# zhenyuw16/Uni3DETR

Hardware: AMD Instinct MI355X
Metric: scenes/sec (fwd+bwd) SUN-RGB-D 20k pts, 300 queries (higher is better)
Workload: dtype bf16

## Files before the change

include/u3d_hip.h:

```cpp
#ifndef U3D_HIP_H_
#define U3D_HIP_H_

#include <stddef.h>
#include <stdint.h>

#ifdef __cplusplus
extern "C" {
#endif

typedef struct ihipStream_t* u3d_stream;

enum {
  U3D_OK = 0,
  U3D_ERR_ARG = -1,
  U3D_ERR_UNSUPPORTED = -2,
  U3D_ERR_LAUNCH = -3,
  U3D_ERR_WORKSPACE = -4
};

enum { U3D_F32 = 0, U3D_BF16 = 1 };

int32_t u3d_version(void);
const char* u3d_strerror(int32_t code);

// ... 54 lines not shown
                           const int32_t* n_out_dev, int32_t n_out_cap, int32_t cin, int32_t cout, int32_t kvol,
                           int32_t transpose_w, u3d_stream s);
int32_t u3d_igemm_fwd_add_bf16(const void* in, const void* w, const int32_t* nbr, int32_t ld, const void* addend, void* out,
                               const int32_t* n_out_dev, int32_t n_out_cap, int32_t cin, int32_t cout, int32_t kvol,
                               int32_t transpose_w, u3d_stream s);
int32_t u3d_linear_bf16(const void* x, const void* w, const float* bias, int32_t relu, void* out, const int32_t* m_dev,
                        int32_t m_cap, int32_t k, int32_t n, u3d_stream s);
int64_t u3d_bn_fold_job_bytes(void);
int32_t u3d_bn_fold_job_blocks(int32_t kvol, int32_t cout, int32_t cin);
int32_t u3d_bn_fold_batched(const void* jobs, int32_t njobs, int32_t total_blocks, u3d_stream s);
int32_t u3d_igemm_fwd_affine_bf16(const void* in, const void* w_folded, const int32_t* nbr, int32_t ld, const float* shift, int32_t relu,
                                  void* out, const int32_t* n_out_dev, int32_t n_out_cap, int32_t cin, int32_t cout, int32_t kvol,
                                  u3d_stream s);
int32_t u3d_igemm_fwd_affine_plan(int32_t n_out_cap, int32_t cin, int32_t cout, int32_t kvol, int32_t has_nbr, int32_t* kernel,
                                  int32_t* rows, int32_t* cols);
int32_t u3d_igemm_fwd_split_bf16(const void* in, const void* w, const int32_t* nbr, int32_t ld, float* out, const int32_t* n_out_dev,
                                 int32_t n_out_cap, int32_t cin, int32_t cout, int32_t kvol3, double* stats, const float* addend, u3d_stream s);
int32_t u3d_igemm_direct_split_bf16(const void* in, const void* w3, const int32_t* nbr, int32_t ld, float* out, const int32_t* n_out_dev,
                                    int32_t n_out_cap, int32_t n_in_cap, int32_t cin, int32_t cout, u3d_stream s);
int32_t u3d_split3_weights(const float* src, int64_t sk, int64_t sa, int64_t sb, int32_t k, int32_t a, int32_t b, void* dst, u3d_stream s);
typedef struct U3dSplitRowsJobs {
  const float* src[32];
  void* dst[32];
  int32_t ld[32], rows[32], cols[32];
  int32_t first_block[33];
  int32_t njobs;
} U3dSplitRowsJobs;
int32_t u3d_split_rows_batch(const U3dSplitRowsJobs* jobs, u3d_stream s);
int32_t u3d_sum3_f32(const float* a, const float* b, const float* c, float* out, int64_t n, u3d_stream s);
int64_t u3d_split3_job_bytes(void);
int32_t u3d_split3_job_blocks(int32_t k, int32_t a, int32_t b);
int32_t u3d_split3_weights_batch(const void* jobs, int32_t njobs, int32_t total_blocks, u3d_stream s);
int32_t u3d_split_rows_f32(const float* x, const int32_t* n_dev, int32_t n_cap, int32_t c, void* dst, u3d_stream s);
int32_t u3d_igemm_fwd_stats_bf16(const void* in, const void* w, const int32_t* nbr, int32_t ld, void* out,
                                 const int32_t* n_out_dev, int32_t n_out_cap, int32_t cin, int32_t cout, int32_t kvol,
                                 double* stats, u3d_stream s);
int32_t u3d_igemm_fwd_stats_layout(int32_t n_out_cap, int32_t cin, int32_t cout, int32_t kvol, int32_t has_nbr, int32_t* partials,
                                   int32_t* rows_per_partial);
typedef struct {
  const void* x;
  const void* y;
  const float* mean;
  const float* invstd;
  const float* gamma;
  const float* beta;
  int32_t relu;
  int32_t reserved;
} u3d_bn_epi;
int32_t u3d_igemm_dgrad_bnstats_bf16(const void* in, const void* w, const int32_t* nbr, int32_t ld, const void* addend, void* out,
                                     const int32_t* n_out_dev, int32_t n_out_cap, int32_t cin, int32_t cout, int32_t kvol,
                                     const u3d_bn_epi* bn, double* stats, u3d_stream s);
int32_t u3d_bn_bwd_finalize_partials(const double* partial, int32_t nblocks, int32_t rows_per_block, const int32_t* n_dev,
                                     int32_t n_cap, int32_t c, double* sums, float* sums_f32, u3d_stream s);
int32_t u3d_subm_halo_sizes(int32_t n_cap, int64_t* tile_rows_elems, int64_t* loc_elems, int32_t* tiles);
int32_t u3d_subm_halo_build(const int32_t* nbr, int32_t ld, const int32_t* n_dev, int32_t n_cap, int32_t* tile_rows,
                            uint16_t* loc, int32_t* tile_cnt, int32_t kvol, u3d_stream s);
int32_t u3d_subm_halo_wpack(const void* w_nmajor, void* w_packed, u3d_stream s);
int32_t u3d_subm_halo_wpack_batched(const void* const* srcs_dev, void* const* dsts_dev, int32_t n, u3d_stream s);
int32_t u3d_subm_halo_conv64_bf16(const void* in, const void* w_packed, const int32_t* tile_rows, const uint16_t* loc,
                                  const int32_t* tile_cnt, const int32_t* n_dev, int32_t n_cap, int32_t krev,
                                  const void* addend, void* out, double* stats, const u3d_bn_epi* bn, int32_t max_slots,
                                  u3d_stream s);
int32_t u3d_subm_halo_wpack128(const void* w_nmajor, void* w_packed, int32_t kvol, u3d_stream s);
int32_t u3d_subm_halo_wpack128_batched(const void* const* srcs_dev, void* const* dsts_dev, int32_t n, int32_t kvol, u3d_stream s);
int32_t u3d_subm_halo_conv128_bf16(const void* in, const void* w_packed, const int32_t* tile_rows, const uint16_t* loc,
                                   const int32_t* tile_cnt, const int32_t* n_dev, int32_t n_cap, int32_t krev,
                                   const void* addend, void* out, double* stats, int32_t max_slots, int32_t kvol, u3d_stream s);
int64_t u3d_subm_halo_wgrad64_workspace(void);
int32_t u3d_subm_halo_wgrad64_bf16(const void* x, const void* dy, const int32_t* tile_rows, const uint16_t* loc,
                                   const int32_t* tile_cnt, const int32_t* n_dev, int32_t n_cap, float* dw, void* workspace,
                                   int64_t workspace_bytes, int32_t max_slots, u3d_stream s);
int64_t u3d_igemm_wgrad_bf16_workspace(int32_t n_out_cap, int32_t cin, int32_t cout, int32_t kvol);
int32_t u3d_igemm_wgrad_bf16(const void* in, const void* dout, const int32_t* nbr, int32_t ld, float* dw,
                             const int32_t* n_out_dev, int32_t n_out_cap, int32_t cin, int32_t cout, int32_t kvol,
                             int32_t out_layout, void* workspace, int64_t workspace_bytes, u3d_stream s);
int32_t u3d_igemm_wgrad_plan(int32_t n_out_cap, int32_t cin, int32_t cout, int32_t kvol, int32_t has_nbr, int32_t out_layout,
                             int32_t* kernel, int32_t* tile, int32_t* nsplit, int64_t* workspace);

int64_t u3d_spconv_wgrad_workspace(int32_t n_out_cap, int32_t cin, int32_t cout, int32_t kvol);
int32_t u3d_spconv_wgrad(const void* in, const void* dout, const int32_t* nbr, int32_t ld, float* dw,
                         const int32_t* n_out_dev, int32_t n_out_cap, int32_t cin, int32_t cout, int32_t kvol,
                         int32_t dtype, void* workspace, int64_t workspace_bytes, u3d_stream s);

int64_t u3d_colsum_workspace(int32_t n, int32_t c);
int32_t u3d_colsum(const void* x, int32_t n, int32_t c, int32_t dtype, float* out, void* workspace,
                   int64_t workspace_bytes, u3d_stream s);

int64_t u3d_wgrad_batched_workspace(int32_t count, int32_t n_rows, int32_t cin, int32_t cout);
int32_t u3d_wgrad_batched_bf16(const void* const* in, const void* const* dout, float* const* dw, int32_t count,
                               const int32_t* n_dev, int32_t n_rows, int32_t cin, int32_t cout, void* workspace,
                               int64_t workspace_bytes, u3d_stream s);
int64_t u3d_colsum_batched_workspace(int32_t count, int32_t n, int32_t c);
int32_t u3d_colsum_batched(const void* const* x, float* const* out, int32_t count, int32_t n, int32_t c, int32_t dtype,
                           void* workspace, int64_t workspace_bytes, u3d_stream s);

int32_t u3d_skinny_wgrad_chunks(int32_t m);
int32_t u3d_skinny_wgrad_bf16(const void* dy, const void* x, int32_t m, int32_t n, int32_t k, float* partial, u3d_stream s);
int32_t u3d_skinny_wgrad_batched(const void* const* dy, const void* const* x, float* const* partial, const int32_t* n, const int32_t* k,
                                 int32_t count, int32_t m, int32_t dy_skinny, u3d_stream s);

int64_t u3d_bn_stats_workspace(int32_t n_cap, int32_t c);
int32_t u3d_bn_stats(const void* x, const int32_t* n_dev, int32_t n_cap, int32_t c, int32_t dtype,
                     double* sums, void* workspace, int64_t workspace_bytes, u3d_stream s);
int32_t u3d_bn_finalize(const double* sums, const int32_t* n_dev, int32_t n_cap, int32_t c, float eps, float momentum,
                        float* running_mean, float* running_var, int64_t* num_batches, float* mean, float* invstd,
                        u3d_stream s);
// ... 367 lines not shown
```

uni3detr_amd/native.py:

```python
import ctypes as C
import os

import numpy as np
import torch

_HERE = os.path.dirname(os.path.abspath(__file__))
LIB_PATH = os.environ.get("U3D_LIB_PATH") or os.path.join(_HERE, "libu3d_hip.so")

F32, BF16 = 0, 1


class U3DError(RuntimeError):
    pass


class BitGridStruct(C.Structure):
    _fields_ = [("words", C.c_void_p), ("prefix", C.c_void_p), ("batch", C.c_int32), ("dz", C.c_int32),
                ("dy", C.c_int32), ("dx", C.c_int32), ("layout", C.c_int32), ("row_capacity", C.c_int32)]


DL_NLIN, DL_NLN = 22, 7
(DL_RPH0, DL_RPH1, DL_RPH2, DL_QS0, DL_QS1, DL_QS2, DL_INQK, DL_INV, DL_OUTP, DL_OPROJ, DL_PE1, DL_FFN0, DL_FFN1, DL_REG0, DL_REG1,
 DL_REG2, DL_CLS0, DL_CLS1, DL_CLS2, DL_IOU0, DL_IOU1, DL_IOU2) = range(DL_NLIN)
(DLN_1, DLN_2, DLN_3, DLN_PE0, DLN_PE1, DLN_C1, DLN_C2) = range(DL_NLN)
# ... 18 lines not shown
    _fields_ = [("src", C.c_void_p), ("dst", C.c_void_p), ("dst_t", C.c_void_p), ("n", C.c_int32), ("k", C.c_int32),
                ("n_pad", C.c_int32), ("n_pad_t", C.c_int32), ("t_plain", C.c_int32), ("reserved", C.c_int32)]


_lib = None
_P = C.c_void_p
_I = C.c_int32
_L = C.c_int64
_I3 = C.c_int32 * 3
_F3 = C.c_float * 3
_F6 = C.c_float * 6

_SIGS = {
    "u3d_version": (_I, []),
    "u3d_strerror": (C.c_char_p, [_I]),
    "u3d_points_augment": (_I, [_P, _P, _I, _I, _I, _P, _I, _I, _P]),
    "u3d_boxes_augment": (_I, [_P, _P, _I, _I, _I, _P, _I, _P]),
    "u3d_points_range_filter": (_I, [_P, _P, _I, _I, C.POINTER(C.c_float), _P, _P, _P]),
    "u3d_point_sample": (_I, [_P, _P, _P, _I, _I, _I, _P, _P, _P, _P]),
    "u3d_boxes_range_filter": (_I, [_P, _P, _P, _I, _I, C.POINTER(C.c_float), _P, _P]),
    "u3d_point_shuffle": (_I, [_P, _P, _P, _I, _I, _I, _P, _P, _P]),
    "u3d_boxes_label_filter": (_I, [_P, _P, _P, _P, _I, _I, _I, _P, _P]),
    "u3d_batch_ingest": (_I, [_P, _I, _I, _P, _P, _I, _I, _P, _I, _I, _P, _P, _P, _I, _I, _P, _P, _P, _P, _P, _P, _P, _P]),
    "u3d_sweeps_merge_workspace": (_L, [_I]),
    "u3d_sweeps_merge": (_I, [_P, _L, _P, _L, _I, _P, _P, _I, _P, _P, _I, _I, C.POINTER(C.c_int32), _I, _I, _P, _L, _P, _L, _P, _P]),
    "u3d_event_create": (_I, [C.POINTER(C.c_void_p)]),
    "u3d_event_record": (_I, [C.c_void_p, _I, _P]),
    "u3d_event_elapsed_ms": (_I, [C.c_void_p, C.c_void_p, C.POINTER(C.c_float)]),
    "u3d_event_destroy": (_I, [C.c_void_p]),
    "u3d_bitgrid_nwords": (_L, [_I, _I, _I, _I]),
    "u3d_bitgrid_nwords_layout": (_L, [_I, _I, _I, _I, _I]),
    "u3d_voxelize_dynamic": (_I, [_P, _P, _I, _I, _I, _F3, _F6, _P, _P]),
    "u3d_scatter_mean": (_I, [_P, _P, _I, _I, _P, _P, _I, _P]),
    "u3d_bitgrid_mark": (_I, [C.POINTER(BitGridStruct), _P, _I, _P]),
    "u3d_bitgrid_mark_strided": (_I, [C.POINTER(BitGridStruct), _P, _P, _I, _I3, _I3, _I3, _P]),
    "u3d_bitgrid_scan_scratch": (_L, [_L]),
    "u3d_bitgrid_scan": (_I, [C.POINTER(BitGridStruct), _P, _P]),
    "u3d_bitgrid_rank": (_I, [C.POINTER(BitGridStruct), _P, _I, _P, _P]),
    "u3d_bitgrid_coords": (_I, [C.POINTER(BitGridStruct), _P, _I, _P]),
    "u3d_nbr_table": (_I, [C.POINTER(BitGridStruct), _P, _P, _I, _I3, _I3, _I3, _I, _P, _I, _P]),
    "u3d_dense_nbr_table": (_I, [_I, _I3, _I3, _I3, _I3, _I3, _I, _P, _I, _P]),
    "u3d_voxelize_hard_workspace": (_L, [_I, _I, _I]),
    "u3d_voxelize_hard": (_I, [_P, _P, _I, _I, _I, _I, _F3, _F6, _I, _I, _P, _P, _P, _P, _P, _P, _L, _P]),
    "u3d_spconv_fwd": (_I, [_P, _P, _P, _I, _P, _P, _I, _I, _I, _I, _I, _I, _P]),
    "u3d_spconv_wgrad_workspace": (_L, [_I, _I, _I, _I]),
    "u3d_spconv_wgrad": (_I, [_P, _P, _P, _I, _P, _P, _I, _I, _I, _I, _I, _P, _L, _P]),
    "u3d_igemm_fwd_bf16": (_I, [_P, _P, _P, _I, _P, _P, _I, _I, _I, _I, _I, _P]),
    "u3d_igemm_fwd_stats_layout": (_I, [_I, _I, _I, _I, _I, _P, _P]),
    "u3d_igemm_fwd_add_bf16": (_I, [_P, _P, _P, _I, _P, _P, _P, _I, _I, _I, _I, _I, _P]),
    "u3d_linear_bf16": (_I, [_P, _P, _P, _I, _P, _P, _I, _I, _I, _P]),
    "u3d_igemm_wgrad_bf16_workspace": (_L, [_I, _I, _I, _I]),
    "u3d_igemm_wgrad_bf16": (_I, [_P, _P, _P, _I, _P, _P, _I, _I, _I, _I, _I, _P, _L, _P]),
    "u3d_igemm_wgrad_plan": (_I, [_I, _I, _I, _I, _I, _I, _P, _P, _P, _P]),
    "u3d_colsum_workspace": (_L, [_I, _I]),
    "u3d_colsum": (_I, [_P, _I, _I, _I, _P, _P, _L, _P]),
    "u3d_bn_stats_workspace": (_L, [_I, _I]),
    "u3d_bn_stats": (_I, [_P, _P, _I, _I, _I, _P, _P, _L, _P]),
    "u3d_bn_finalize": (_I, [_P, _P, _I, _I, C.c_float, C.c_float, _P, _P, _P, _P, _P, _P]),
    "u3d_bn_forward_stats": (_I, [_P, _P, _I, _I, _I, C.c_float, C.c_float, _P, _P, _P, _P, _P, _P, _L, _P]),
    "u3d_bn_finalize_partials": (_I, [_P, _I, _I, _P, _I, _I, C.c_float, C.c_float, _P, _P, _P, _P, _P, _P]),
    "u3d_igemm_fwd_stats_bf16": (_I, [_P, _P, _P, _I, _P, _P, _I, _I, _I, _I, _P, _P]),
    "u3d_igemm_fwd_split_bf16": (_I, [_P, _P, _P, _I, _P, _P, _I, _I, _I, _I, _P, _P, _P]),
    "u3d_split_rows_f32": (_I, [_P, _P, _I, _I, _P, _P]),
    "u3d_split3_weights": (_I, [_P, C.c_int64, C.c_int64, C.c_int64, _I, _I, _I, _P, _P]),
    "u3d_sum3_f32": (_I, [_P, _P, _P, _P, C.c_int64, _P]),
    "u3d_split_rows_batch": (_I, [_P, _P]),
    "u3d_split3_job_bytes": (C.c_int64, []),
    "u3d_split3_job_blocks": (_I, [_I, _I, _I]),
    "u3d_split3_weights_batch": (_I, [_P, _I, _I, _P]),
    "u3d_bn_fold_job_bytes": (C.c_int64, []),
    "u3d_bn_fold_job_blocks": (_I, [_I, _I, _I]),
    "u3d_bn_fold_batched": (_I, [_P, _I, _I, _P]),
    "u3d_igemm_fwd_affine_bf16": (_I, [_P, _P, _P, _I, _P, _I, _P, _P, _I, _I, _I, _I, _P]),
    "u3d_igemm_fwd_affine_plan": (_I, [_I, _I, _I, _I, _I, _P, _P, _P]),
    "u3d_igemm_direct_split_bf16": (_I, [_P, _P, _P, _I, _P, _P, _I, _I, _I, _I, _P]),
    "u3d_igemm_dgrad_bnstats_bf16": (_I, [_P, _P, _P, _I, _P, _P, _P, _I, _I, _I, _I, _P, _P, _P]),
    "u3d_bn_bwd_finalize_partials": (_I, [_P, _I, _I, _P, _I, _I, _P, _P, _P]),
    "u3d_subm_halo_sizes": (_I, [_I, _P, _P, _P]),
    "u3d_subm_halo_build": (_I, [_P, _I, _P, _I, _P, _P, _P, _I, _P]),
    "u3d_subm_halo_wpack128": (_I, [_P, _P, _I, _P]),
    "u3d_subm_halo_wpack128_batched": (_I, [_P, _P, _I, _I, _P]),
    "u3d_subm_halo_conv128_bf16": (_I, [_P, _P, _P, _P, _P, _P, _I, _I, _P, _P, _P, _I, _I, _P]),
    "u3d_subm_halo_wgrad64_workspace": (_L, []),
    "u3d_subm_halo_wgrad64_bf16": (_I, [_P, _P, _P, _P, _P, _P, _I, _P, _P, _L, _I, _P]),
    "u3d_subm_halo_wpack": (_I, [_P, _P, _P]),
    "u3d_subm_halo_wpack_batched": (_I, [_P, _P, _I, _P]),
    "u3d_subm_halo_conv64_bf16": (_I, [_P, _P, _P, _P, _P, _P, _I, _I, _P, _P, _P, _P, _I, _P]),
    "u3d_bn_apply": (_I, [_P, _P, _P, _P, _P, _P, _I, _P, _P, _I, _I, _I, _P, _P, _P]),
    "u3d_bn_bwd_stats": (_I, [_P, _P, _P, _P, _P, _P, _P, _I, _P, _I, _I, _I, _P, _P, _L, _P, _P, _P]),
    "u3d_bn_bwd_apply": (_I, [_P, _P, _P, _P, _P, _P, _P, _P, _I, _P, _P, _P, _I, _I, _I, _P, _P]),
    "u3d_bn_apply_planes": (_I, [_P, _P, _P, _P, _P, _P, _I, _P, _P, _P, _I, _I, _P, _P, _P]),
    "u3d_bn_bwd_apply_planes": (_I, [_P, _P, _P, _P, _P, _P, _P, _P, _I, _P, _P, _P, _P, _I, _I, _P, _P]),
    "u3d_to_dense": (_I, [_P, _P, _P, _I, _I, _P, _I, _I, _I, _I, _P]),
    "u3d_from_dense": (_I, [_P, _P, _P, _I, _I, _P, _I, _I, _I, _I, _P]),
    "u3d_fps": (_I, [_P, _P, _P, _I, _I, _I, _P, _P, _L, _P, _L, _I, _P]),
    "u3d_refine_decode_fwd": (_I, [_P, _P, _P, _I, _I, _P, C.c_float, _P, _P, _P, _P]),
    "u3d_loss_targets": (_I, [_P, _P, _P, _P, _I, _I, _I, _I, _I, _P, _P, _P, _P, _P, _P]),
    "u3d_fps2": (_I, [_P, _P, _I, _P, _P, _I, _I, _I, _P, _P, _L, _P, _L, _I, _P]),
    "u3d_fps_prep": (_I, [_P, _I, _P, _P, _I, _I, _P, _P, _P, _P]),
    "u3d_fps_points": (_I, [_P, _I, _P, _P, _P, _P, _I, _I, _P, _P]),
    "u3d_query_embed_fwd": (_I, [_P, _P, _P, _P, _I, _I, _I, _I, _P, _P, _P, _P, _P]),
    "u3d_query_embed_bwd": (_I, [_P, _P, _P, _P, _P, _I, _I, _I, _I, _P, _P, _P]),
    "u3d_match_cost": (_I, [_P, _P, _P, _P, _P, _I, _I, _I, _I, _I, _I, C.c_float, C.c_float, C.c_float, C.c_float, C.c_float, _P, _P]),
    "u3d_lsa": (_I, [_P, _P, _I, _I, _I, _I, _I, _P, _P]),
    "u3d_trilinear_fwd": (_I, [_P, _P, _I, _I, _I, _I, _I, _I, _P, _I, _P]),
    "u3d_trilinear_bwd": (_I, [_P, _P, _P, _I, _I, _I, _I, _I, _I, _P, _P, _I, _P]),
# ... 505 lines not shown
    def ptr_ld(self):
        k, ld = self.t.shape
        return C.c_void_p(self.t.data_ptr() + (k - 1) * ld * 4), -ld


def _nbr_ptr_ld(nbr):
    if nbr is None:
        return _ptr(None), 0
    if isinstance(nbr, RevNbr):
        return nbr.ptr_ld()
    return _ptr(nbr), nbr.shape[1]


def spconv_fwd(inp, w, nbr, n_out_dev, n_out, cout, transpose_w=False, tag=None, addend=None):
    kvol = w.shape[0]
    cin = inp.shape[1]
    out = torch.empty((n_out, cout), dtype=inp.dtype, device=inp.device)
    nbr_p, ld = _nbr_ptr_ld(nbr)
    if isinstance(nbr, RevNbr):
        nbr = nbr.t.flip(0) if (TIMER is not None and TIMER.mode == "census") else None
    t = TIMER
    e0 = t.begin() if t is not None else None
    rc = -2
    if addend is not None and inp.dtype == torch.bfloat16 and USE_IGEMM_V2 and ld != 0 and addend.dtype == torch.bfloat16 \
            and addend.shape == out.shape and addend.is_contiguous():
        rc = lib().u3d_igemm_fwd_add_bf16(_ptr(inp), _ptr(w), nbr_p, ld, _ptr(addend), _ptr(out), _ptr(n_out_dev), n_out, cin, cout, kvol,
                                          1 if transpose_w else 0, _stream())
        if rc not in (0, -2):
            _check(rc, "igemm_fwd_add_bf16")
        if rc == 0:
            addend = None
    if rc == -2 and inp.dtype == torch.bfloat16 and USE_IGEMM_V2:
        rc = lib().u3d_igemm_fwd_bf16(_ptr(inp), _ptr(w), nbr_p, ld, _ptr(out), _ptr(n_out_dev), n_out, cin, cout, kvol,
                                      1 if transpose_w else 0, _stream())
        if rc not in (0, -2):
            _check(rc, "igemm_fwd_bf16")
    if rc == -2:
        _check(lib().u3d_spconv_fwd(_ptr(inp), _ptr(w), nbr_p, ld, _ptr(out), _ptr(n_out_dev), n_out, cin, cout, kvol,
                                    1 if transpose_w else 0, dtype_code(inp), _stream()), "spconv_fwd")
    if t is not None:
        meta = None
        if t.mode == "census":
            pairs = int((nbr[:, :n_out] >= 0).sum().item()) if nbr is not None else n_out
            s = inp.element_size()
            meta = dict(kind=CALL_KIND, v2=bool(rc == 0), n_in=inp.shape[0], n_out=n_out, cin=cin, cout=cout, kvol=kvol, pairs=pairs,
                        bytes=inp.shape[0] * cin * s + n_out * cout * s + 8 * pairs + kvol * cin * cout * s,
                        flops=2 * pairs * cin * cout)
        t.end(tag or ("spconv_dgrad" if transpose_w else "spconv_fwd"), e0, meta)
    if addend is not None:
        out += addend
    return out


def split_rows(x, n_dev, n_cap=None):
    n_cap = x.shape[0] if n_cap is None else n_cap
    assert x.dtype == torch.float32 and x.is_contiguous()
    out = torch.empty((2 * n_cap, x.shape[1]), dtype=torch.bfloat16, device=x.device)
    _check(lib().u3d_split_rows_f32(_ptr(x), _ptr(n_dev), n_cap, x.shape[1], _ptr(out), _stream()), "split_rows_f32")
    return out


def direct_serves(cin, cout, kvol):
    return kvol == 27 and cin in (16, 32, 64) and cout in (16, 32, 64) and not (cin == 64 and cout == 64)


def spconv_fwd_split_direct(xs, w3, nbr, n_out_dev, n_out, cout, tag="spconv_fwd"):
    cin, n_in = xs.shape[1], xs.shape[0] // 2
    out = torch.empty((n_out, cout), dtype=torch.float32, device=xs.device)
    nbr_p, ld = _nbr_ptr_ld(nbr)
    t = TIMER
    e0 = t.begin() if t is not None else None
    _check(lib().u3d_igemm_direct_split_bf16(_ptr(xs), _ptr(w3), nbr_p, ld, _ptr(out), _ptr(n_out_dev), n_out, n_in, cin, cout, _stream()),
           "igemm_direct_split_bf16")
    if t is not None:
        meta = None
        if t.mode == "census":
            tab = nbr.t.flip(0) if isinstance(nbr, RevNbr) else nbr
            pairs = int((tab[:, :n_out] >= 0).sum().item())
            meta = dict(kind=CALL_KIND, v2=True, split=True, n_in=n_in, n_out=n_out, cin=cin, cout=cout, kvol=27, pairs=pairs,
                        bytes=n_in * cin * 4 + n_out * cout * 4 + 8 * pairs + 27 * cin * cout * 4, flops=2 * pairs * cin * cout)
        t.end(tag, e0, meta)
    return out


class _SplitRowsJobs(C.Structure):
    _fields_ = [("src", C.c_void_p * 32), ("dst", C.c_void_p * 32), ("ld", C.c_int32 * 32), ("rows", C.c_int32 * 32), ("cols", C.c_int32 * 32),
                ("first_block", C.c_int32 * 33), ("njobs", C.c_int32)]


def split_rows_batch_into(tensors, outs):
    for i in range(0, len(tensors), 32):
        jobs = _SplitRowsJobs()
        chunk = list(zip(tensors[i:i + 32], outs[i:i + 32]))
        jobs.njobs = len(chunk)
        for j, (t, o) in enumerate(chunk):
            assert t.dtype == torch.float32 and t.dim() == 2 and t.stride(1) == 1 and t.shape[1] % 4 == 0 and t.stride(0) % 4 == 0
            assert o.dtype == torch.bfloat16 and o.is_contiguous() and tuple(o.shape) == (2 * t.shape[0], t.shape[1])
            jobs.src[j], jobs.dst[j] = t.data_ptr(), o.data_ptr()
            jobs.ld[j], jobs.rows[j], jobs.cols[j] = t.stride(0), t.shape[0], t.shape[1]
        _check(lib().u3d_split_rows_batch(C.byref(jobs), _stream()), "split_rows_batch")


def split_rows_batch(tensors):
    outs = [torch.empty((2 * t.shape[0], t.shape[1]), dtype=torch.bfloat16, device=t.device) for t in tensors]
    split_rows_batch_into(tensors, outs)
    return outs
# ... 1488 lines not shown
```

uni3detr_amd/plugin/dense.py:

```python

import numpy as np
import torch
from torch import nn

from .. import native as nv
from .. import sparse as sp
from ..registry import BACKBONES, NECKS


def _conv(cfg, cin, cout, kernel, stride=1, padding=0):
    cfg = dict(cfg)
    t = cfg.pop("type")
    if t != "Conv3d":
        raise NotImplementedError("the HIP dense path implements the Conv3d variant used by every shipped config")
    if cfg.get("bias", True):
        raise NotImplementedError("shipped configs build these convolutions with bias=False")
    return nn.Conv3d(cin, cout, kernel, stride=stride, padding=padding, **cfg)


def _norm(cfg, c):
    cfg = dict(cfg)
    t = cfg.pop("type")
    assert t == "BN3d", "shipped configs use BN3d"
    cfg.pop("requires_grad", None)
    return nn.BatchNorm3d(c, **cfg)


_BRANCH_STREAMS = []
PARALLEL_BRANCHES = True


class Lattice:

    _cache = {}

    @classmethod
    def conv(cls, device, batch, dims_in, ksize, stride, pad):
        key = ("c", str(device), batch, tuple(dims_in), tuple(ksize), tuple(stride), tuple(pad))
        g = cls._cache.get(key)
        if g is None:
            dims_out = tuple((d + 2 * p - k) // s + 1 for d, k, s, p in zip(dims_in, ksize, stride, pad))
            n_in = batch * dims_in[0] * dims_in[1] * dims_in[2]
            n_out = batch * dims_out[0] * dims_out[1] * dims_out[2]
            one = all(k == 1 for k in ksize) and all(s == 1 for s in stride)
            fwd = None if one else nv.dense_nbr_table(batch, dims_out, dims_in, ksize, stride, pad, 0, device)
            bwd = None if one else nv.dense_nbr_table(batch, dims_in, dims_out, ksize, stride, pad, 1, device)
            n_in_dev = torch.tensor([n_in], dtype=torch.int32, device=device)
            n_out_dev = torch.tensor([n_out], dtype=torch.int32, device=device)
            g = (sp.ConvGeom(fwd, bwd, n_in, n_in_dev, n_out, n_out_dev, kind="dense", strided=any(s > 1 for s in stride)), dims_out)
            cls._cache[key] = g
        return g

    @classmethod
    def upsample_index(cls, device, batch, dims_in, s):
        key = ("u", str(device), batch, tuple(dims_in), s)
        v = cls._cache.get(key)
        if v is None:
            D, H, W = dims_in
            b = torch.arange(batch, device=device).view(-1, 1, 1, 1)
            z = torch.arange(D, device=device).view(1, -1, 1, 1)
            y = torch.arange(H * s, device=device).view(1, 1, -1, 1)
            x = torch.arange(W * s, device=device).view(1, 1, 1, -1)
            in_row = ((b * D + z) * H + y // s) * W + x // s
            tap = (y % s) * s + (x % s)
            idx = (in_row * (s * s) + tap).reshape(-1).int().contiguous()
            inv = torch.empty_like(idx)
            inv[idx.long()] = torch.arange(idx.numel(), device=device, dtype=torch.int32)
            v = (idx, inv, (D, H * s, W * s))
            cls._cache[key] = v
        return v


FUSED_LEVEL_SUM = True
FUSED_UPSAMPLE_ORDER = True


class _GatherBijection(torch.autograd.Function):
    @staticmethod
    def forward(ctx, rows, idx, inv):
        ctx.save_for_backward(inv)
        return nv.gather_rows(rows.contiguous(), idx)

    @staticmethod
    def backward(ctx, dout):
        (inv,) = ctx.saved_tensors
        return nv.gather_rows(dout.contiguous(), inv), None, None


def to_rows(x):
    B, C, D, H, W = x.shape
    return x.permute(0, 2, 3, 4, 1).reshape(-1, C), B, (D, H, W)


def to_volume(rows, B, dims):
    return rows.view(B, *dims, rows.shape[1]).permute(0, 4, 1, 2, 3)


def conv_bn_relu(rows, B, dims, conv, bn, post_add=None, fan_token=None, bn_in=None, bn_out=None):
    ks, st, pd = tuple(conv.kernel_size), tuple(conv.stride), tuple(conv.padding)
    geom, dims_out = Lattice.conv(rows.device, B, dims, ks, st, pd)
    return sp.conv_bn(rows, conv.weight, geom, bn, geom.n_out_dev, None, True, "oidhw", post_add, fan_token=fan_token, bn_in=bn_in,
                      bn_out=bn_out), dims_out
# ... 137 lines not shown
```

uni3detr_amd/sparse.py:

```python
import contextlib
import os

import torch

from . import native as nv
from .shadow import conv_weights, halo_packs

K3, S1, P1 = (3, 3, 3), (1, 1, 1), (1, 1, 1)


class Level:

    def __init__(self, grid, coords, n, n_dev):
        self.grid, self.coords, self.n, self.n_dev = grid, coords, n, n_dev
        self.dims, self.batch = grid.dims, grid.batch
        self._subm = None
        self._halo = None

    def halo(self):
        if self._halo is None:
            h = nv.SubmHalo(self.subm_tables()[0], self.n_dev, self.n) if self.n <= nv.SubmHalo.MAX_ROWS else None
            self._halo = h if (h is not None and h.ok) else False
        return self._halo or None

    def subm_tables(self):
        if self._subm is None:
            fwd = self.grid.nbr_table(self.coords, self.n_dev, K3, S1, P1, 0)
            bwd = nv.RevNbr(fwd) if REV_SUBM_TABLE else self.grid.nbr_table(self.coords, self.n_dev, K3, S1, P1, 1)
            self._subm = (fwd, bwd)
        return self._subm


class ResidualToken:

    def __init__(self):
        self.dres = None


class BnGradToken:

    def __init__(self):
        self.epi = None
        self.keep = None
        self.partial = None
        self.c = 0

    def fill(self, x, y, mean, invstd, gamma, beta, relu):
        self.keep = (x, y, mean, invstd, gamma, beta)
        self.epi = nv.BnEpi.of(x, y, mean, invstd, gamma, beta, relu)
        self.c = x.shape[1]


class FanoutToken:

    def __init__(self, n):
        self.n = self.remaining = n
        self.acc = None

    def step(self, din):
        self.remaining -= 1
        if self.remaining > 0:
            self.acc = din
            return None
        self.acc, self.remaining = None, self.n
        return din


class ConvGeom:

    def __init__(self, nbr_fwd, nbr_bwd, n_in, n_in_dev, n_out, n_out_dev, kind="sparse", strided=False):
        self.strided = strided
        self.nbr_fwd, self.nbr_bwd = nbr_fwd, nbr_bwd
        self.n_in, self.n_in_dev, self.n_out, self.n_out_dev = n_in, n_in_dev, n_out, n_out_dev
        self.kind = kind
        self.level = None


def level_from_coors(coors, batch, dims):
    dev = coors.device
    g = nv.BitGrid(batch, dims, dev)
    g.mark(coors)
    g.scan()
    n = coors.shape[0]
    g.set_row_capacity(n)
    rank = g.rank(coors)
    lvl = Level(g, g.coords(n), n, g.count_dev)
    return lvl, rank


def subm_geom(lvl):
    fwd, bwd = lvl.subm_tables()
    g = ConvGeom(fwd, bwd, lvl.n, lvl.n_dev, lvl.n, lvl.n_dev)
    g.level = lvl
    return g


def strided_level(lvl, ksize, stride, pad, capacity=None):
    dims_out = tuple((d + 2 * p - k) // s + 1 for d, k, s, p in zip(lvl.dims, ksize, stride, pad))
    g = nv.BitGrid(lvl.batch, dims_out, lvl.coords.device)
    g.mark_strided(lvl.coords, lvl.n_dev, ksize, stride, pad)
    g.scan()
    n_out = int(g.count_dev.item()) if capacity is None else int(capacity)
    if capacity is not None:
        g.set_row_capacity(n_out)
    out = Level(g, g.coords(n_out), n_out, g.count_dev)
    fwd = lvl.grid.nbr_table(out.coords, out.n_dev, ksize, stride, pad, 0)
    bwd = g.nbr_table(lvl.coords, lvl.n_dev, ksize, stride, pad, 1)
    return out, ConvGeom(fwd, bwd, lvl.n, lvl.n_dev, n_out, out.n_dev, strided=True)


REV_SUBM_TABLE = True
SUBM_HALO = os.environ.get("U3D_SUBM_HALO", "1") == "1"
HALO_WGRAD = True
HALO_128 = True
STRIDED_DGRAD_SPLIT = True
NMAJOR_FWD = True
STRIDED_SPLIT_MIN_RATIO = 16
STRIDED_SPLIT_SPARSE_RATIO = 16


_CONV_USES = {}


def reset_conv_uses():
    _CONV_USES.clear()
    _PLANES_BWD.clear()


SPLIT_BF16 = os.environ.get("U3D_SPLIT_BF16", "1") == "1"
SPLIT_FUSED_ADD = True
_SPLIT = [False]


_PLANES = {}
_PLANES_BWD = {}
BN_PLANES = True


def _planes_of(feats, n_dev):
    ent = _PLANES.get(id(feats))
    if ent is not None and ent[0] is feats and ent[2] == feats._version:
        return ent[1]
    xs = nv.split_rows(feats.contiguous(), n_dev)
    if _SPLIT[0]:
        _PLANES[id(feats)] = (feats, xs, feats._version)
    return xs


def _give_planes(t, planes):
    if planes is not None and _SPLIT[0]:
        _PLANES[id(t)] = (t, planes, t._version)


def _give_bwd_planes(t, planes):
    if planes is not None:
        _PLANES_BWD[t.data_ptr()] = (t, planes, t._version)


def _bwd_planes_of(dout, n_dev):
    ent = _PLANES_BWD.pop(dout.data_ptr(), None)
    if (ent is not None and ent[0].numel() == dout.numel() and ent[0].dtype == dout.dtype and ent[2] == ent[0]._version
            and dout.dim() == 2 and dout.is_contiguous() and ent[0].is_contiguous()):
        return ent[1].view(2 * dout.shape[0], dout.shape[1])
    return nv.split_rows(dout.float() if dout.dtype != torch.float32 else dout, n_dev)


@contextlib.contextmanager
def split_scope(on=True, split3=None):
    prev, prev3 = _SPLIT[0], nv.SPLIT3_ACTIVE
    _SPLIT[0] = bool(on) and SPLIT_BF16
    _PLANES.clear()
# ... 49 lines not shown
        split = _split_serves(feats, cin, cout, kv)
        if split == "narrow" and geom.nbr_fwd is None:
            split = None
        kio, koi = (None, None) if split else conv_weights(weight, layout, feats.dtype, want_koi=nmajor)
        ctx.geom, ctx.layout = geom, layout
        ctx.res_token = res_token
        ctx.fan_token = fan_token if (fan_token is not None and feats.requires_grad) else None
        ctx.bn_in = bn_in if (BN_GRAD_FUSION and bn_in is not None and bn_in.epi is not None and bf16 and fan_token is None) else None
        _CONV_USES[id(weight)] = _CONV_USES.get(id(weight), 0) + 1
        ctx.weight_id = id(weight)
        ctx.grad_view = getattr(weight, "_u3d_grad_view", None)
        ctx.kio_shape, ctx.wdtype = kio_shape, weight.dtype
        nv.CALL_KIND = geom.kind
        ctx.split = split
        if ctx.split:
            n_in = feats.shape[0]
            xs = _planes_of(feats, geom.n_in_dev)
            ctx.save_for_backward(xs, weight)
            ctx.halo = False
            ctx.split3 = nv.SPLIT3_ACTIVE
            w3 = nv.split3_weights(weight, layout, nmajor=True)
            if split == "narrow":
                y = nv.spconv_fwd_split_direct(xs, w3, geom.nbr_fwd, geom.n_out_dev, geom.n_out, cout)
                res = (y, None, 0)
            else:
                t3 = _split_table(geom, "fwd", geom.n_out, n_in)
                res = nv.spconv_fwd_split(xs, w3, t3, geom.n_out_dev, geom.n_out, cout, want_stats=want_stats)
                if not want_stats:
                    return res
            if not want_stats:
                return res[0]
            y, stats, tr = res
            if stats is None:
                stats = torch.empty(0, dtype=torch.float64, device=feats.device)
            else:
                stats._u3d_tile_rows = tr
            ctx.mark_non_differentiable(stats)
            return y, stats
        ctx.halo = False
        ctx.save_for_backward(feats, kio)
        nbr = geom.nbr_fwd if kio.shape[0] > 1 else None
        ctx.halo = (SUBM_HALO and REV_SUBM_TABLE and nmajor and geom.level is not None and kv == 27 and cin == cout
                    and (cin == 64 or (cin == 128 and HALO_128)) and geom.n_out >= 4096
                    and geom.level.halo() is not None)
        ctx.halo_tab = geom.level.halo() if ctx.halo else None
        if ctx.halo:
            pk_fwd, ctx.pk_bwd = halo_packs(weight, kio, koi)
            if want_stats:
                y, stats, tr = nv.subm_halo_conv(feats, pk_fwd, ctx.halo_tab, want_stats=True)
                stats._u3d_tile_rows = tr
                ctx.mark_non_differentiable(stats)
                return y, stats
            return nv.subm_halo_conv(feats, pk_fwd, ctx.halo_tab)
        if want_stats:
            res = nv.spconv_fwd_stats(feats, koi, nbr, geom.n_out_dev, geom.n_out, cout) if nmajor else None
            if res is not None:
                y, stats, tr = res
                stats._u3d_tile_rows = tr
            else:
                y = (nv.spconv_fwd(feats, koi, nbr, geom.n_out_dev, geom.n_out, cout, transpose_w=True, tag="spconv_fwd") if nmajor
                     else nv.spconv_fwd(feats, kio, nbr, geom.n_out_dev, geom.n_out, cout))
                stats = torch.empty(0, dtype=torch.float64, device=feats.device)
            ctx.mark_non_differentiable(stats)
            return y, stats
        if nmajor:
            return nv.spconv_fwd(feats, koi, nbr, geom.n_out_dev, geom.n_out, cout, transpose_w=True, tag="spconv_fwd")
        return nv.spconv_fwd(feats, kio, nbr, geom.n_out_dev, geom.n_out, cout)

    @staticmethod
    def backward(ctx, dout, _dstats=None):
        feats, wc = ctx.saved_tensors
        g = ctx.geom
        if dout is None:
            return None, None, None, None, None, None, None, None
        dout = dout.contiguous()
        kvol = wc.shape[0]
        din = dw = None
        nv.CALL_KIND = g.kind
        if ctx.split:
            return _SparseConv._split_backward(ctx, feats, wc, dout)

        def weight_grad():
            nbr = g.nbr_fwd if kvol > 1 else None
            cin_w, cout_w = wc.shape[1], wc.shape[2]
            v2 = feats.dtype == torch.bfloat16 and nv.USE_IGEMM_V2 and cin_w % 16 == 0 and cout_w % 16 == 0 and ctx.wdtype == torch.float32
            gv = ctx.grad_view if (v2 and ctx.grad_view is not None and ctx.grad_view.is_contiguous()
                                   and ctx.grad_view.dtype == torch.float32 and _CONV_USES.get(ctx.weight_id, 0) == 1) else None
            if ctx.layout == "oidhw" and v2:
                ks = ctx.kio_shape
                dw = nv.spconv_wgrad(feats, dout, nbr, g.n_out_dev, kvol, out_oik=True, out=gv).view(ks[4], ks[3], ks[0], ks[1], ks[2])
            elif ctx.layout == "dhwio" and v2 and ctx.halo and HALO_WGRAD and cin_w == 64:
                dw = nv.subm_halo_wgrad(feats, dout, ctx.halo_tab, out=gv).view(ctx.kio_shape)
            elif ctx.layout == "dhwio" and v2:
                dw = nv.spconv_wgrad(feats, dout, nbr, g.n_out_dev, kvol, out=gv).view(ctx.kio_shape)
            else:
                dw = nv.spconv_wgrad(feats, dout, nbr, g.n_out_dev, kvol).reshape(ctx.kio_shape).to(ctx.wdtype)
                if ctx.layout == "oidhw":
                    dw = dw.permute(4, 3, 0, 1, 2)
            return dw

        if ctx.needs_input_grad[1]:
            dw = weight_grad()
        if ctx.needs_input_grad[0]:
            nbr = g.nbr_bwd if kvol > 1 else None
            cin, cout = wc.shape[1], wc.shape[2]
            fan = ctx.fan_token
            facc = fan.acc if fan is not None else None
            if (STRIDED_DGRAD_SPLIT and g.strided and kvol > 1 and dout.dtype == torch.bfloat16 and cout % 64 == 0
                    and (kvol * cin) % 64 == 0
                    and g.n_out * (STRIDED_SPLIT_SPARSE_RATIO if g.kind == "sparse" else STRIDED_SPLIT_MIN_RATIO) <= g.n_in):
                prod = nv.linear_bf16(dout, wc.view(kvol * cin, cout), None, False)
                fa = facc if (facc is not None and facc.dtype == prod.dtype and facc.is_contiguous() and facc.shape == (g.n_in, cin)) else None
                din = nv.tap_gather_sum(prod, nbr, g.n_in_dev, g.n_in, cin, kvol, addend=fa)
                if facc is not None and fa is None:
                    din += facc
            else:
                tok = ctx.res_token
                add = tok.dres if tok is not None else None
                if tok is not None:
                    tok.dres = None
                if add is not None and facc is not None:
                    add = add + facc
                elif facc is not None:
                    add = facc
                bt = ctx.bn_in
                if bt is not None and (bt.c != cin or (add is not None and not (add.dtype == torch.bfloat16 and add.is_contiguous()))):
                    bt = None
                if ctx.halo and cin != 64:
                    bt = None
                if ctx.halo:
                    pk = ctx.pk_bwd if ctx.pk_bwd is not None else nv.subm_halo_wpack(wc)
                    if bt is not None:
                        din, st, tr = nv.subm_halo_conv(dout, pk, ctx.halo_tab, krev=True, addend=add, want_stats=True, tag="spconv_dgrad",
                                                        bn_epi=bt.epi)
                        bt.partial = (st, tr)
                    else:
                        din = nv.subm_halo_conv(dout, pk, ctx.halo_tab, krev=True, addend=add, tag="spconv_dgrad")
                else:
                    r = nv.spconv_dgrad_bnstats(dout, wc, nbr, g.n_in_dev, g.n_in, cin, add, bt.epi) if (bt is not None and kvol > 1) else None
                    if r is not None:
                        din, bt.partial = r[0], (r[1], r[2])
                    else:
                        din = nv.spconv_fwd(dout, wc, nbr, g.n_in_dev, g.n_in, cin, transpose_w=True, addend=add)
            if fan is not None:
                din = fan.step(din)
        elif ctx.res_token is not None:
            ctx.res_token.dres = None
        return din, dw, None, None, None, None, None, None


def _split_backward_impl(ctx, xs, wc, dout):
    g = ctx.geom
    ks = ctx.kio_shape
    kvol, cin, cout = ks[0] * ks[1] * ks[2], ks[3], ks[4]
    n_in, n_out = xs.shape[0] // 2, dout.shape[0]
    dys = _bwd_planes_of(dout, g.n_out_dev)
    din = dw = None
    if ctx.split == "narrow":
        if ctx.needs_input_grad[1]:
            xh, xl, dyh, dyl = xs[:n_in], xs[n_in:], dys[:n_out], dys[n_out:]
            dwk = nv.sum3(nv.spconv_wgrad(xh, dyh, g.nbr_fwd, g.n_out_dev, kvol), nv.spconv_wgrad(xl, dyh, g.nbr_fwd, g.n_out_dev, kvol),
                          nv.spconv_wgrad(xh, dyl, g.nbr_fwd, g.n_out_dev, kvol)).reshape(ctx.kio_shape).to(ctx.wdtype)
            dw = dwk.permute(4, 3, 0, 1, 2) if ctx.layout == "oidhw" else dwk
        if ctx.needs_input_grad[0]:
            din = nv.spconv_fwd_split_direct(dys, nv.split3_weights(wc, ctx.layout, nmajor=False, cache=getattr(ctx, "split3", None)), g.nbr_bwd, g.n_in_dev, g.n_in, cin,
                                             tag="spconv_dgrad")
            fan, tok = ctx.fan_token, ctx.res_token
            if fan is not None:
                if fan.acc is not None:
                    din += fan.acc
                din = fan.step(din)
            if tok is not None and tok.dres is not None:
                din = din + tok.dres
                tok.dres = None
        elif ctx.res_token is not None:
            ctx.res_token.dres = None
        return din, dw, None, None, None, None, None, None
    if ctx.needs_input_grad[1]:
        ta = _split_table(g, "wgrad", n_out, n_in)
        tb = ta[:kvol]
        a = nv.spconv_wgrad(xs, dys[:n_out], ta, g.n_out_dev, 2 * kvol)
        b = nv.spconv_wgrad(xs, dys[n_out:], tb, g.n_out_dev, kvol)
        dwk = nv.sum3(a[:kvol], a[kvol:], b).reshape(ctx.kio_shape).to(ctx.wdtype)
        dw = dwk.permute(4, 3, 0, 1, 2) if ctx.layout == "oidhw" else dwk
    if ctx.needs_input_grad[0]:
        if (STRIDED_DGRAD_SPLIT and g.strided and kvol > 1 and (kvol * cin) % 64 == 0
                and n_out * (STRIDED_SPLIT_SPARSE_RATIO if g.kind == "sparse" else STRIDED_SPLIT_MIN_RATIO) <= g.n_in):
            tid = _split_table(g, "id", n_out, n_out)
            wt3 = nv.split3_weights(wc, ctx.layout, nmajor=False, cache=getattr(ctx, "split3", None)).view(3, kvol * cin, cout)
            prod = nv.spconv_fwd_split(dys, wt3, tid, g.n_out_dev, n_out, kvol * cin, tag="spconv_dgrad")
# ... 190 lines not shown
```

Baseline: 422.0.

## Add dense window conv kernel for 1x3x3 dense 128-channel layers

Adds a specialised HIP kernel for dense 1x3x3 stride-1 128→128 convolutions. It loads a contiguous raster halo of input rows into LDS once per 256-row tile and derives the neighbour offsets from the raster shift, so no gather through a neighbour table is needed. Weights are double-buffered through LDS and boundary taps are masked. It is wired into the forward and dgrad paths (optionally fusing the addend) for dense geometries that record raster metadata. The cost is large LDS use per block, which can lower occupancy, and the path only applies to that narrow shape.

```diff
diff --git a/include/u3d_hip.h b/include/u3d_hip.h
--- a/include/u3d_hip.h
+++ b/include/u3d_hip.h
@@ -130,6 +130,11 @@
                                      const u3d_bn_epi* bn, double* stats, u3d_stream s);
 int32_t u3d_bn_bwd_finalize_partials(const double* partial, int32_t nblocks, int32_t rows_per_block, const int32_t* n_dev,
                                      int32_t n_cap, int32_t c, double* sums, float* sums_f32, u3d_stream s);
+int32_t u3d_dense_window_plan(int32_t n_cap, int32_t H, int32_t W, int32_t cin, int32_t cout, const int32_t ksize[3],
+                              const int32_t stride[3], const int32_t pad[3], int32_t* tile_rows, int32_t* stats_blocks,
+                              int64_t* lds_bytes);
+int32_t u3d_dense_window_conv_bf16(const void* in, const void* w_nmajor, int32_t planes, int32_t H, int32_t W, int32_t reverse,
+                                   const void* addend, void* out, double* stats, const int32_t* n_dev, int32_t n_cap, u3d_stream s);
 int32_t u3d_subm_halo_sizes(int32_t n_cap, int64_t* tile_rows_elems, int64_t* loc_elems, int32_t* tiles);
 int32_t u3d_subm_halo_build(const int32_t* nbr, int32_t ld, const int32_t* n_dev, int32_t n_cap, int32_t* tile_rows,
                             uint16_t* loc, int32_t* tile_cnt, int32_t kvol, u3d_stream s);
diff --git a/uni3detr_amd/csrc/dense_window.hip b/uni3detr_amd/csrc/dense_window.hip
--- /dev/null
+++ b/uni3detr_amd/csrc/dense_window.hip
@@ -0,0 +1,197 @@
+#include "igemm_common.h"
+
+namespace {
+struct BnEpi {
+  static constexpr const u16* x = nullptr;
+};
+template <int BM, int BN, int NT>
+__device__ __forceinline__ void bn_bwd_tile_sums(const BnEpi, u16*, int, int, int, int, int, double*, int) {}
+
+constexpr int DW_BM = 256, DW_C = 128, DW_NW = 8;
+constexpr int DW_WBUF = 2 * DW_C * 64;
+constexpr int DW_MAX_ROWS = (1 << 23) - 1;
+
+struct DwPlan {
+  int tile_rows = 0, blocks = 0;
+  size_t lds = 0;
+};
+}
+
+__global__ __launch_bounds__(DW_NW * 64) void k_dense_window_128(const u16* __restrict__ in, const u16* __restrict__ w, int planes, int H,
+                                                                 int W, int reverse, const float* __restrict__ bias, int relu,
+                                                                 u16* __restrict__ out, double* __restrict__ stats,
+                                                                 const int* __restrict__ n_dev, int n_cap) {
+  constexpr int NW = DW_NW, WAVES_M = 4, WAVES_N = 2, WM = 4, WN = 4;
+  constexpr int BM = DW_BM, BN = DW_C;
+  constexpr bool F32OUT = false;
+  extern __shared__ __attribute__((aligned(16))) u16 smem[];
+  u16* const Wb = smem;
+  u16* const R = smem + 2 * DW_WBUF;
+
+  const int n_out = min(min(*n_dev, n_cap), planes * H * W);
+  const int tile = u3d_xcd_tile(blockIdx.x, (n_out + BM - 1) / BM);
+  if (tile < 0) return;
+  const int m0 = tile * BM;
+  const int col0 = 0, cout = DW_C;
+  const int tid = threadIdx.x, lane = tid & 63;
+  const int wv = __builtin_amdgcn_readfirstlane(tid >> 6);
+  const int wm = wv / WAVES_N, wn = wv % WAVES_N;
+  const BnEpi bn;
+
+  f32x4 acc[WM][WN];
+#pragma unroll
+  for (int a = 0; a < WM; ++a)
+#pragma unroll
+    for (int b = 0; b < WN; ++b) acc[a][b] = (f32x4){0.f, 0.f, 0.f, 0.f};
+
+  const __amdgpu_buffer_rsrc_t in_rs = __builtin_amdgcn_make_buffer_rsrc((void*)in, 0, n_out * (DW_C * 2), 0x00020000);
+  const __amdgpu_buffer_rsrc_t w_rs = __builtin_amdgcn_make_buffer_rsrc((void*)w, 0, 9 * DW_C * DW_C * 2, 0x00020000);
+
+  unsigned w_voff[2];
+#pragma unroll
+  for (int u = 0; u < 2; ++u) {
+    const int r = (wv * 2 + u) * 8 + (lane >> 3);
+    const int part = (lane & 7) ^ ((r >> 1) & 7);
+    w_voff[u] = (unsigned)(r * DW_C + part * 8) * 2u;
+  }
+  auto issue_w = [&](int pair, int buf) {
+#pragma unroll
+    for (int h = 0; h < 2; ++h) {
+      const int st = 2 * pair + h, kap = st % 9, c = st / 9;
+      const unsigned soff = (unsigned)(kap * DW_C * DW_C + c * 64) * 2u;
+      u16* dst = Wb + buf * DW_WBUF + h * (DW_C * 64) + wv * 1024;
+#pragma unroll
+      for (int u = 0; u < 2; ++u) __builtin_amdgcn_raw_ptr_buffer_load_lds(w_rs, (lds_void_ptr)(dst + u * 512), 16, w_voff[u], soff, 0, 0);
+    }
+  };
+  issue_w(0, 0);
+
+  const int run = BM + 2 * W + 2;
+  {
+    const int ni = (run + 3) >> 2;
+    const int lrow = lane >> 4, lslot = lane & 15;
+    for (int q = wv; q < ni; q += NW) {
+      const int rb = min(q * 4, run - 4);
+      const int r = rb + lrow;
+      const int grow = m0 - W - 1 + r;
+      const unsigned voff = (grow >= 0 && grow < n_out) ? (unsigned)grow * (DW_C * 2u) + (unsigned)(lslot ^ (r & 15)) * 16u : 0xFFFFFFFFu;
+      __builtin_amdgcn_raw_ptr_buffer_load_lds(in_rs, (lds_void_ptr)(R + rb * DW_C), 16, voff, 0, 0, 0);
+    }
+  }
+
+  const int g = lane >> 4, li = lane & 15, fsw = (lane >> 1) & 7;
+  typedef const volatile s16x8 __attribute__((address_space(3))) * lds_vptr;
+  int wfoff[2];
+#pragma unroll
+  for (int ks = 0; ks < 2; ++ks) wfoff[ks] = ((ks * 4 + g) ^ fsw) << 3;
+
+  unsigned amask[WM];
+#pragma unroll
+  for (int a = 0; a < WM; ++a) {
+    const int m = m0 + (wm * WM + a) * 16 + li;
+    const int x = m % W, y = (m / W) % H;
+    unsigned bits = 0;
+#pragma unroll
+    for (int kap = 0; kap < 9; ++kap) {
+      const int dy = reverse ? 1 - kap / 3 : kap / 3 - 1, dx = reverse ? 1 - kap % 3 : kap % 3 - 1;
+      if ((unsigned)(y + dy) < (unsigned)H && (unsigned)(x + dx) < (unsigned)W) bits |= 1u << kap;
+    }
+    amask[a] = bits;
+  }
+  const int arow0 = wm * WM * 16 + li + W + 1;
+
+  auto load_a = [&](int pair, int t, bf16x8 (&af)[WM]) {
+    const int st = 2 * pair + (t >> 1), kap = st % 9, c = st / 9, ks = t & 1;
+    const int shift = ((kap / 3 - 1) * W + (kap % 3 - 1)) * (reverse ? -1 : 1);
+    const int rr = arow0 + shift;
+    const int key = rr & 15;
+    const u16* Ap = R + rr * DW_C + (((c * 8 + ks * 4 + g) ^ key) << 3);
+#pragma unroll
+    for (int a = 0; a < WM; ++a) {
+      s16x8 v = *(lds_vptr)(Ap + a * 16 * DW_C);
+      if (!((amask[a] >> kap) & 1u)) v = (s16x8){0, 0, 0, 0, 0, 0, 0, 0};
+      af[a] = __builtin_bit_cast(bf16x8, v);
+    }
+  };
+  auto load_w = [&](int buf, int t, bf16x8 (&wf)[WN]) {
+    const u16* Wp = Wb + buf * DW_WBUF + (t >> 1) * (DW_C * 64) + (wn * WN * 16 + li) * 64 + wfoff[t & 1];
+#pragma unroll
+    for (int b = 0; b < WN; ++b) {
+      const s16x8 v = *(lds_vptr)(Wp + b * 16 * 64);
+      wf[b] = __builtin_bit_cast(bf16x8, v);
+    }
+  };
+
+  __builtin_amdgcn_s_waitcnt(0x0F70);
+  __syncthreads();
+  bf16x8 af[2][WM], wf[2][WN];
+  load_a(0, 0, af[0]);
+  load_w(0, 0, wf[0]);
+#pragma unroll 1
+  for (int pair = 0; pair < 9; ++pair) {
+    const int buf = pair & 1;
+    if (pair + 1 < 9) issue_w(pair + 1, buf ^ 1);
+#pragma unroll
+    for (int t = 0; t < 4; ++t) {
+      const int cur = t & 1;
+      if (t < 3) {
+        load_a(pair, t + 1, af[cur ^ 1]);
+        load_w(buf, t + 1, wf[cur ^ 1]);
+      } else if (pair + 1 < 9) {
+        load_a(pair + 1, 0, af[cur ^ 1]);
+      }
+#pragma unroll
+      for (int b = 0; b < WN; ++b)
+#pragma unroll
+        for (int a = 0; a < WM; ++a) acc[a][b] = __builtin_amdgcn_mfma_f32_16x16x32_bf16(wf[cur][b], af[cur][a], acc[a][b], 0, 0, 0);
+    }
+    __builtin_amdgcn_s_waitcnt(0x0F70);
+    __syncthreads();
+    if (pair + 1 < 9) load_w(buf ^ 1, 0, wf[0]);
+  }
+#define GLDS_EPI_ADDEND 1
+#include "glds_epilogue.inc"
+#undef GLDS_EPI_ADDEND
+}
+
+static int dense_window_plan(int n_cap, int H, int W, int cin, int cout, const int32_t ksize[3], const int32_t stride[3],
+                             const int32_t pad[3], DwPlan* p) {
+  if (ksize[0] != 1 || ksize[1] != 3 || ksize[2] != 3 || stride[0] != 1 || stride[1] != 1 || stride[2] != 1 || pad[0] != 0 ||
+      pad[1] != 1 || pad[2] != 1 || cin != DW_C || cout != DW_C || H <= 0 || W <= 0 || n_cap < 0 || n_cap > DW_MAX_ROWS)
+    return U3D_ERR_UNSUPPORTED;
+  const size_t lds = (size_t)(DW_BM + 2 * W + 2) * (DW_C * 2) + 2 * (size_t)DW_WBUF * 2;
+  if (lds > 160 * 1024) return U3D_ERR_UNSUPPORTED;
+  p->tile_rows = DW_BM;
+  p->blocks = u3d_cdiv(n_cap, DW_BM);
+  p->lds = lds;
+  return U3D_OK;
+}
+
+extern "C" int32_t u3d_dense_window_plan(int32_t n_cap, int32_t H, int32_t W, int32_t cin, int32_t cout, const int32_t ksize[3],
+                                         const int32_t stride[3], const int32_t pad[3], int32_t* tile_rows, int32_t* stats_blocks,
+                                         int64_t* lds_bytes) {
+  U3D_REQUIRE(ksize && stride && pad && tile_rows && stats_blocks && lds_bytes, U3D_ERR_ARG);
+  DwPlan p;
+  const int rc = dense_window_plan(n_cap, H, W, cin, cout, ksize, stride, pad, &p);
+  if (rc != U3D_OK) return rc;
+  *tile_rows = p.tile_rows;
+  *stats_blocks = p.blocks;
+  *lds_bytes = (int64_t)p.lds;
+  return U3D_OK;
+}
+
+extern "C" int32_t u3d_dense_window_conv_bf16(const void* in, const void* w_nmajor, int32_t planes, int32_t H, int32_t W, int32_t reverse,
+                                              const void* addend, void* out, double* stats, const int32_t* n_dev, int32_t n_cap,
+                                              u3d_stream s) {
+  U3D_REQUIRE(in && w_nmajor && out && n_dev && planes > 0 && H > 0 && W > 0, U3D_ERR_ARG);
+  U3D_REQUIRE((long long)planes * H * W <= DW_MAX_ROWS, U3D_ERR_UNSUPPORTED);
+  const int32_t k133[3] = {1, 3, 3}, s111[3] = {1, 1, 1}, p011[3] = {0, 1, 1};
+  DwPlan p;
+  const int rc = dense_window_plan(n_cap, H, W, DW_C, DW_C, k133, s111, p011, &p);
+  if (rc != U3D_OK) return rc;
+  if (p.blocks == 0) return U3D_OK;
+  U3D_ALLOW_LDS(k_dense_window_128, 160 * 1024);
+  hipLaunchKernelGGL(k_dense_window_128, dim3(p.blocks), dim3(DW_NW * 64), p.lds, (hipStream_t)s, (const u16*)in, (const u16*)w_nmajor,
+                     planes, H, W, reverse ? 1 : 0, (const float*)addend, addend ? 2 : 0, (u16*)out, stats, n_dev, n_cap);
+  return hipGetLastError() == hipSuccess ? U3D_OK : U3D_ERR_LAUNCH;
+}
diff --git a/uni3detr_amd/native.py b/uni3detr_amd/native.py
--- a/uni3detr_amd/native.py
+++ b/uni3detr_amd/native.py
@@ -94,6 +94,8 @@
     "u3d_igemm_wgrad_bf16_workspace": (_L, [_I, _I, _I, _I]),
     "u3d_igemm_wgrad_bf16": (_I, [_P, _P, _P, _I, _P, _P, _I, _I, _I, _I, _I, _P, _L, _P]),
     "u3d_igemm_wgrad_plan": (_I, [_I, _I, _I, _I, _I, _I, _P, _P, _P, _P]),
+    "u3d_dense_window_plan": (_I, [_I, _I, _I, _I, _I, _I3, _I3, _I3, _P, _P, _P]),
+    "u3d_dense_window_conv_bf16": (_I, [_P, _P, _I, _I, _I, _I, _P, _P, _P, _P, _I, _P]),
     "u3d_colsum_workspace": (_L, [_I, _I]),
     "u3d_colsum": (_I, [_P, _I, _I, _I, _P, _P, _L, _P]),
     "u3d_bn_stats_workspace": (_L, [_I, _I]),
@@ -705,6 +707,39 @@
     return out
 
 
+def dense_window_plan(n_cap, H, W, cin, cout, ksize, stride, pad):
+    tr, nb, lds = C.c_int32(0), C.c_int32(0), C.c_int64(0)
+    if lib().u3d_dense_window_plan(n_cap, H, W, cin, cout, _I3(*ksize), _I3(*stride), _I3(*pad), C.byref(tr), C.byref(nb),
+                                   C.byref(lds)) != 0:
+        return None
+    return tr.value, nb.value, lds.value
+
+
+def dense_window_conv(inp, w_nmajor, raster, n_dev, n, reverse=False, addend=None, want_stats=False, tag=None):
+    planes, H, W, ksize, stride, pad = raster
+    cin, cout, kvol = inp.shape[1], w_nmajor.shape[1], w_nmajor.shape[0]
+    plan = dense_window_plan(n, H, W, cin, cout, ksize, stride, pad)
+    if plan is None or inp.dtype != torch.bfloat16 or w_nmajor.dtype != torch.bfloat16 or kvol != 9:
+        raise U3DError(f"dense_window_conv: shape not served ({cin} -> {cout}, kernel {ksize}, stride {stride}, pad {pad}, W = {W})")
+    tile_rows, blocks, _ = plan
+    out = torch.empty((n, cout), dtype=inp.dtype, device=inp.device)
+    stats = torch.empty((blocks, 2, cout), dtype=torch.float64, device=inp.device) if want_stats else None
+    if addend is not None:
+        assert addend.dtype == torch.bfloat16 and addend.shape == out.shape and addend.is_contiguous()
+    t = TIMER
+    e0 = t.begin() if t is not None else None
+    _check(lib().u3d_dense_window_conv_bf16(_ptr(inp), _ptr(w_nmajor), planes, H, W, 1 if reverse else 0, _ptr(addend), _ptr(out),
+                                            _ptr(stats), _ptr(n_dev), n, _stream()), "dense_window_conv_bf16")
+    if t is not None:
+        meta = None
+        if t.mode == "census":
+            pairs = planes * sum((H - abs(dy)) * (W - abs(dx)) for dy in (-1, 0, 1) for dx in (-1, 0, 1))
+            meta = dict(kind=CALL_KIND, v2=True, n_in=inp.shape[0], n_out=n, cin=cin, cout=cout, kvol=kvol, pairs=pairs,
+                        bytes=inp.shape[0] * cin * 2 + n * cout * 2 + 8 * pairs + kvol * cin * cout * 2, flops=2 * pairs * cin * cout)
+        t.end(tag or ("spconv_dgrad" if reverse else "spconv_fwd"), e0, meta)
+    return (out, stats, tile_rows) if want_stats else out
+
+
 def split_rows(x, n_dev, n_cap=None):
     n_cap = x.shape[0] if n_cap is None else n_cap
     assert x.dtype == torch.float32 and x.is_contiguous()
diff --git a/uni3detr_amd/plugin/dense.py b/uni3detr_amd/plugin/dense.py
--- a/uni3detr_amd/plugin/dense.py
+++ b/uni3detr_amd/plugin/dense.py
@@ -48,6 +48,7 @@
             n_in_dev = torch.tensor([n_in], dtype=torch.int32, device=device)
             n_out_dev = torch.tensor([n_out], dtype=torch.int32, device=device)
             g = (sp.ConvGeom(fwd, bwd, n_in, n_in_dev, n_out, n_out_dev, kind="dense", strided=any(s > 1 for s in stride)), dims_out)
+            g[0].raster = (batch * dims_in[0], dims_in[1], dims_in[2], tuple(ksize), tuple(stride), tuple(pad))
             cls._cache[key] = g
         return g
 
diff --git a/uni3detr_amd/sparse.py b/uni3detr_amd/sparse.py
--- a/uni3detr_amd/sparse.py
+++ b/uni3detr_amd/sparse.py
@@ -74,6 +74,8 @@
         self.n_in, self.n_in_dev, self.n_out, self.n_out_dev = n_in, n_in_dev, n_out, n_out_dev
         self.kind = kind
         self.level = None
+        self.raster = None
+        self._window = {}
 
 
 def level_from_coors(coors, batch, dims):
@@ -113,10 +115,22 @@
 SUBM_HALO = os.environ.get("U3D_SUBM_HALO", "1") == "1"
 HALO_WGRAD = True
 HALO_128 = True
+DENSE_WINDOW = True
 STRIDED_DGRAD_SPLIT = True
 NMAJOR_FWD = True
 STRIDED_SPLIT_MIN_RATIO = 16
 STRIDED_SPLIT_SPARSE_RATIO = 16
+
+
+def window_serves(geom, cin, cout):
+    if geom.raster is None:
+        return False
+    ok = geom._window.get((cin, cout))
+    if ok is None:
+        _, H, W, ks, st, pd = geom.raster
+        ok = geom.n_in == geom.n_out and nv.dense_window_plan(geom.n_out, H, W, cin, cout, ks, st, pd) is not None
+        geom._window[(cin, cout)] = ok
+    return ok
 
 
 _CONV_USES = {}
@@ -272,6 +286,15 @@
                 ctx.mark_non_differentiable(stats)
                 return y, stats
             return nv.subm_halo_conv(feats, pk_fwd, ctx.halo_tab)
+        ctx.window = bool(DENSE_WINDOW and nmajor and not ctx.halo and koi is not None and koi.dtype == torch.bfloat16
+                          and kio.dtype == torch.bfloat16 and window_serves(geom, cin, cout))
+        if ctx.window:
+            if want_stats:
+                y, stats, tr = nv.dense_window_conv(feats, koi, geom.raster, geom.n_out_dev, geom.n_out, want_stats=True)
+                stats._u3d_tile_rows = tr
+                ctx.mark_non_differentiable(stats)
+                return y, stats
+            return nv.dense_window_conv(feats, koi, geom.raster, geom.n_out_dev, geom.n_out)
         if want_stats:
             res = nv.spconv_fwd_stats(feats, koi, nbr, geom.n_out_dev, geom.n_out, cout) if nmajor else None
             if res is not None:
@@ -356,6 +379,11 @@
                         bt.partial = (st, tr)
                     else:
                         din = nv.subm_halo_conv(dout, pk, ctx.halo_tab, krev=True, addend=add, tag="spconv_dgrad")
+                elif ctx.window and bt is None and dout.dtype == torch.bfloat16:
+                    fused = add is not None and add.dtype == torch.bfloat16 and add.is_contiguous() and tuple(add.shape) == (g.n_in, cin)
+                    din = nv.dense_window_conv(dout, wc, g.raster, g.n_in_dev, g.n_in, reverse=True, addend=add if fused else None)
+                    if add is not None and not fused:
+                        din += add
                 else:
                     r = nv.spconv_dgrad_bnstats(dout, wc, nbr, g.n_in_dev, g.n_in, cin, add, bt.epi) if (bt is not None and kvol > 1) else None
                     if r is not None:
```

Result: no change. 423.5, median of 6 (+0.4%).
